# microsoft/foldingdiff

Measured on AMD Instinct MI355X. Metric: backbones/sec (L=128, T=1000, bs=512), higher is better.
Workload: dtype f32 (fp16 hi/lo split operands, 3x v_mfma_f32_{32x32x16,16x16x32}_f16 per product, fp32 accumulate)

## Files before the change

foldingdiff_amd/build.py:

```python
import os
import shutil
import subprocess
import sys
from concurrent.futures import ThreadPoolExecutor

PKG_DIR = os.path.dirname(os.path.abspath(__file__))
CSRC = os.path.join(PKG_DIR, "csrc")
LIB_DIR = os.path.join(PKG_DIR, "_lib")
LIB_PATH = os.path.join(LIB_DIR, "libfdmi.so")
SOURCES = ["api.hip", "api_weights.hip", "api_comm.hip", "api_run.hip", "api_structures.hip", "api_hooks.hip", "gemm_f32.hip", "gemm_img.hip", "gemm_ws.hip", "gemm_ln_rows.hip", "attention_f32.hip", "attention_img.hip", "attention_gen.hip", "seq_attn.hip", "seq_attn16.hip", "ffn16.hip", "rowwise.hip",
           "rowwise_img.hip", "inpaint_jump.hip", "loss.hip", "loss_variants.hip", "nerf.hip", "internal_coords.hip", "tm_score.hip", "psea.hip", "dssp.hip", "tm_align.hip", "tm_align_starts.hip", "clash_lddt.hip", "angle_stats.hip", "steer.hip", "repeat_tie.hip", "nerf_vjp.hip", "nerf_scan.hip", "relax.hip", "guide_scaffold.hip", "template_fit.hip"]
HEADERS = [os.path.join(CSRC, "fdmi_kernels.h"), os.path.join(CSRC, "img_common.h"), os.path.join(CSRC, "horn_fit.h"),
           os.path.join(CSRC, "launch_common.h"), os.path.join(CSRC, "host_common.h"), os.path.join(CSRC, "model.h"), os.path.join(CSRC, "weight_pack.h"), os.path.join(CSRC, "tm_search.h"), os.path.join(CSRC, "tm_align_common.h"), os.path.join(CSRC, "wrap_pi.h"), os.path.join(CSRC, "nerf_place.h"), os.path.join(CSRC, "smooth_l1_term.h"), os.path.join(CSRC, "philox_normal.h"), os.path.join(CSRC, "inpaint_replace.h"), os.path.join(CSRC, "strided_update.h"), os.path.join(CSRC, "solver_update.h"), os.path.join(CSRC, "p_sample_update.h"), os.path.join(CSRC, "block_sum.h"), os.path.join(CSRC, "guide_element.h"), os.path.join(os.path.dirname(PKG_DIR), "include", "fdmi.h")]
ARCH = "gfx950"
PER_SOURCE_FLAGS = {
    "attention_img": ["-fno-slp-vectorize"],
    "attention_gen": ["-fno-slp-vectorize"],
    "seq_attn": ["-fno-slp-vectorize"],
    "seq_attn16": ["-fno-slp-vectorize"],
    "ffn16": ["-fno-slp-vectorize"],
}
CXXFLAGS = ["-O3", "-std=c++17", "-fPIC", f"--offload-arch={ARCH}", "-Wall", "-Wno-unused-function"]


def find_hipcc() -> str:
    for cand in (os.environ.get("HIPCC"), shutil.which("hipcc"), "/opt/rocm/bin/hipcc"):
        if cand and os.path.exists(cand):
            return cand
    raise RuntimeError("hipcc not found (set HIPCC=/path/to/hipcc)")


def _stale(target: str, deps) -> bool:
    if not os.path.exists(target):
        return True
    t = os.path.getmtime(target)
    return any(os.path.getmtime(d) > t for d in deps)


def build(force: bool = False, verbose: bool = False, variant: str = "", defines=()) -> str:
    hipcc = find_hipcc()
    os.makedirs(LIB_DIR, exist_ok=True)
    lib_dir = os.path.join(LIB_DIR, variant) if variant else LIB_DIR
    lib_path = os.path.join(lib_dir, "libfdmi.so")
    obj_dir = os.path.join(lib_dir, "obj")
    os.makedirs(obj_dir, exist_ok=True)
    jobs = []
    objs = []
    revs = dict(d[4:].split("=", 1) for d in defines if d.startswith("rev:"))
    defines = [d for d in defines if not d.startswith("rev:")]
    old_sources = []
    for src in SOURCES:
        sp = os.path.join(CSRC, src)
        if src in revs:
# ... 6 lines not shown
        op = os.path.join(obj_dir, src.replace(".hip", ".o"))
        objs.append(op)
        if force or _stale(op, [sp] + HEADERS):
            stem = src.replace(".hip", "")
            extra = [d.split("=", 1)[1] for d in defines if d.startswith("@") and d[1:].split("=", 1)[0] in (stem, "all")]
            jobs.append([hipcc] + CXXFLAGS + PER_SOURCE_FLAGS.get(stem, []) + extra
                        + [f"-D{d}" for d in defines if not d.startswith("@")] + ["-c", sp, "-o", op])

    def run(cmd):
        if verbose:
            print(" ".join(cmd), flush=True)
        r = subprocess.run(cmd, capture_output=True, text=True)
        if r.returncode != 0:
            raise RuntimeError(f"hipcc failed ({r.returncode}):\n{' '.join(cmd)}\n{r.stdout}\n{r.stderr}")
        return r

    try:
        with ThreadPoolExecutor(max_workers=8) as ex:
            list(ex.map(run, jobs))
        counts = mfma_counts(defines, {src: os.path.join(CSRC, f"_rev_{variant}_{src}") for src in revs}) if variant else None
    finally:
        for sp in old_sources:
            os.remove(sp)
    if force or jobs or _stale(lib_path, objs):
        run([hipcc, f"--offload-arch={ARCH}", "-shared", "-fPIC"] + objs + ["-o", lib_path])
    if variant:
        import json
        meta = {"defines": list(defines), "revs": revs, "mfma": counts, "mfma_default": mfma_counts(())}
        with open(os.path.join(lib_dir, "build_info.json"), "w") as fh:
            json.dump(meta, fh, indent=1, sort_keys=True)
    return lib_path


MFMA_SOURCES = ["seq_attn16.hip", "ffn16.hip", "seq_attn.hip", "gemm_img.hip", "attention_img.hip"]


def mfma_counts(defines=(), paths=None) -> dict:
    import re
    import tempfile
    hipcc = find_hipcc()
    out = {}
    with tempfile.TemporaryDirectory() as td:
        for src in MFMA_SOURCES:
            stem = src.replace(".hip", "")
            extra = [d.split("=", 1)[1] for d in defines if d.startswith("@") and d[1:].split("=", 1)[0] in (stem, "all")]
            asm = os.path.join(td, stem + ".s")
            cmd = [hipcc, "-O3", "-std=c++17", f"--offload-arch={ARCH}", "-Wno-unused-function"] + PER_SOURCE_FLAGS.get(stem, []) + extra \
                + [f"-D{d}" for d in defines if not d.startswith("@")] + ["-S", "--cuda-device-only", "-o", asm, (paths or {}).get(src, os.path.join(CSRC, src))]
            r = subprocess.run(cmd, capture_output=True, text=True)
            if r.returncode != 0:
                raise RuntimeError(f"hipcc -S failed for {src}:\n{r.stderr[-2000:]}")
            text = open(asm).read()
            for m in re.finditer(r"^(_Z\w+):[^\n]*\n(.*?)^\.Lfunc_end\d+:", text, re.S | re.M):
                n = m.group(2).count("v_mfma")
                if n:
                    out[m.group(1)] = n
    return out


if __name__ == "__main__":
    args = [a for a in sys.argv[1:] if a != "--force"]
    p = build(force="--force" in sys.argv, verbose=True, variant=args[0] if args else "", defines=args[1:])
    print(p)
```

foldingdiff_amd/csrc/api.hip:

```cpp
#include <hip/hip_runtime.h>

#include <cstdarg>
#include <cstdio>
#include <cstring>
#include <string>
#include <utility>
#include <vector>

#include "../../include/fdmi.h"
#include "fdmi_kernels.h"
#include "host_common.h"
#include "launch_common.h"
#include "model.h"

using namespace fdmi;

namespace {
thread_local std::string g_err;
}

int fdmi::fail(int code, const char* fmt, ...) {
  char buf[1024];
  va_list ap;
  va_start(ap, fmt);
// ... 174 lines not shown
  m->pending.clear();
  return FD_OK;
}

#define PROF(cls, stmt)                                   \
  do {                                                    \
    int rc_ = prof_begin(m, cls, s, mode.profile);        \
    if (rc_) return rc_;                                  \
    stmt;                                                 \
    rc_ = prof_end(m, s, mode.profile);                   \
    if (rc_) return rc_;                                  \
  } while (0)

void prof_drop(fd_model* m, bool on) {
  if (!on) return;
  const PendingEvent p = m->pending.back();
  m->pending.pop_back();
  m->event_pool.push_back(p.e0);
  m->event_pool.push_back(p.e1);
}

struct EnvOverrides {
  int fuse_attn, fuse_ffn;
  bool stamps;
};
const EnvOverrides& env_overrides() {
  static const EnvOverrides env = [] {
    auto num = [](const char* name, int dflt) { const char* e = getenv(name); return e ? atoi(e) : dflt; };
    return EnvOverrides{num("FDMI_FUSE_ATTN", -1), num("FDMI_FUSE_FFN", -1), num("FDMI_STAMPS", 0) != 0};
  }();
  return env;
}

}

StepPlan fdmi::plan_step(const fd_model* m, const Workspace& w, bool key_mask, bool dyn_rows) {
  StepPlan p;
  p.img = w.img;
  if (!p.img) {
    p.fuse_ln = m->fuse_ln > 0;
    return p;
  }
  const fd_config& c = m->cfg;
  const LayerDev& lw = m->layers[0];
  const EnvOverrides& env = env_overrides();
  const int B = w.B, L = w.L, d = c.d_model, max_rows = w.cap, ncu = cu_count();
  auto whole_rounds = [&](int items) {
    const int rounds = (items + ncu - 1) / ncu;
    return (double)items >= 0.94 * (double)rounds * ncu;
  };
  const bool fits_u32 = (size_t)w.cap * d * 4 < (1ull << 32) - 65536;
  const int fuse_attn = m->fuse_attn >= 0 ? m->fuse_attn : env.fuse_attn;
  const bool attn_auto = !m->varlen && L > 96 && whole_rounds(B);
  const bool fused_ok = fuse_attn != 0 && (fuse_attn > 0 || attn_auto) && !key_mask && !m->split_qkv && fits_u32;
  if (fused_ok && fuse_attn != 2 && lw.wsa16_i.p && seq_attn16_supported(d, c.n_heads, L, c.max_pos)) p.attn = StepPlan::ATTN_FUSED16;
  else if (fused_ok && fuse_attn == 2 && lw.wsa_i.p && seq_attn_supported(d, c.n_heads, L, c.max_pos)) p.attn = StepPlan::ATTN_FUSED32;
  else p.attn = lw.wqkv_i.p && !m->split_qkv ? StepPlan::ATTN_QKV : StepPlan::ATTN_QK_VT;
  p.attn_gen = key_mask || head_dim(c) != 32;
  const int fuse_ffn = m->fuse_ffn >= 0 ? m->fuse_ffn : env.fuse_ffn;
  const int rows_known = m->varlen && m->rows_hint > 0 && m->rows_hint <= max_rows ? m->rows_hint : max_rows;
  const bool fused_ffn = fuse_ffn != 0 && (fuse_ffn > 0 || whole_rounds((rows_known + 127) / 128)) && lw.wff_i.p &&
                         ffn16_supported(d, c.d_ff) && fits_u32;
  p.ffn = !fused_ffn ? StepPlan::FFN_GEMMS : (fuse_ffn != 1 && lw.wtail_i.p && d <= 384) ? StepPlan::FFN_TAIL : StepPlan::FFN_FUSED;
  p.split_ln = d > 384;
  auto tail_for = [&](int N) {
    if (m->varlen || dyn_rows) return 1;
    const int ntiles = (max_rows / 128) * ((N + 383) / 384);
    return ntiles % gemm_img_grid(max_rows, N) != 0 ? 1 : 0;
  };
  if (!p.fused_attn()) p.tail_qk = tail_for(p.attn == StepPlan::ATTN_QKV ? 3 * d : 2 * d);
  p.tail_d = tail_for(d);
  if (p.ffn == StepPlan::FFN_GEMMS) p.tail_ff = tail_for(c.d_ff);
  return p;
}

namespace {

UpdateArgs fill_update(const fd_model* m, const Workspace& w, const StepMode& mode) {
  UpdateArgs u;
  memset(&u, 0, sizeof u);
  if (m->cfg.decoder == FD_DEC_MLP) {
    u.gamma = m->hd_g;
    u.beta = m->hd_b;
    u.do_ln = 1;
  }
  u.w2 = m->hd_w2;
  u.b2 = m->hd_b2;
  u.x = w.x;
  u.coef = m->coef;
  u.t_dev = w.t_dev;
  u.T = m->T;
  u.M = w.B * w.L;
  u.L = w.L;
  u.F = m->cfg.n_features;
  u.d = m->cfg.d_model;
  u.ln_eps = 1e-12f;
// ... 157 lines not shown
        PROF(KC_GEMM_QKV, launch_gemm_img(EPI_IMG_QK, g, max_rows, s));
        if (stop_after(1)) return done();
        g = base();
        g.A = w.himg; g.W = static_cast<const unsigned char*>(lw.wv_i.p); g.bias = lw.bv;
        g.vbuf = w.vbuf; g.N = d; g.K = d;
        g.acc_scale = 1.0f / (lw.s_h * lw.wv_i.scale); g.v_scale = lw.s_v;
        g.tail = plan.tail_d;
        PROF(KC_GEMM_V, launch_gemm_img(EPI_IMG_VT, g, max_rows, s));
        if (stop_after(1)) return done();
      }
      AttnImgArgs a;
      memset(&a, 0, sizeof a);
      a.qbuf = w.qbuf; a.kbuf = w.kbuf; a.vbuf = w.vbuf;
      a.demb = static_cast<const u32x4_t*>(lw.demb_s.p);
      a.lens = w.lens; a.nrow = w.nrow; a.seq_row0 = w.seq_row0; a.ctx = w.cimg; a.trash = w.trash;
      a.B = B; a.H = H; a.LTOT = w.LTOT; a.NKT = w.NKT; a.maxpos = c.max_pos;
      a.q_scale = lw.s_q; a.k_scale = lw.s_k; a.v_scale = lw.s_v; a.ctx_scale = lw.s_v;
      a.r_scale = lw.demb_s.p ? lw.s_k / lw.demb_s.scale : 1.f;
      a.r_scale_k = lw.demb_s.p ? lw.s_q / lw.demb_s.scale : 1.f;
      a.rkq = c.pos_type == FD_POS_RELATIVE_KEY_QUERY;
      a.stamps = stamps_at(kStampAttn);
      bool ok = true;
      if (plan.attn_gen) {
        a.H = c.n_heads;
        a.kmask = mode.kmask;
        a.L = mode.kmask ? L : 0;
        PROF(KC_ATTN, ok = launch_attention_gen(a, head_dim(c) / 32, s));
      } else {
        PROF(KC_ATTN, ok = launch_attention_img(a, L, s));
      }
      if (!ok) return fail(FD_E_UNSUPPORTED, "attention: L=%d, head size %d", L, head_dim(c));
      if (stop_after(1)) return done();
    }
    const bool fused_tail = plan.ffn == StepPlan::FFN_TAIL;
    if (!fused_tail) {
      GemmImgArgs g = base();
      g.A = w.cimg; g.W = static_cast<const unsigned char*>(lw.wo_i.p); g.bias = lw.bo; g.gamma = lw.ln1g; g.beta = lw.ln1b;
      g.resid = w.himg; g.out = w.aimg; g.K = d;
      g.acc_scale = 1.0f / (lw.s_v * lw.wo_i.scale); g.resid_inv = 1.0f / lw.s_h; g.out_scale = lw.s_a;
      if (int rc = gemm_ln(g, KC_GEMM_OUT, KC_LN1)) return rc;
      if (stop_after(1)) return done();
    }
    if (plan.ffn != StepPlan::FFN_GEMMS) {
      FfnArgs a;
      memset(&a, 0, sizeof a);
      a.aimg = w.aimg; a.a_bytes = (unsigned)((size_t)w.cap * d * 4);
      a.wimg = static_cast<const unsigned char*>(fused_tail ? lw.wtail_i.p : lw.wff_i.p);
      if (fused_tail) {
        a.cimg = w.cimg; a.hres = w.himg; a.bo = lw.bo; a.g1 = lw.ln1g; a.b1 = lw.ln1b;
        a.ao_scale = 1.0f / (lw.s_v * lw.wtail_i.scale); a.hres_inv = 1.0f / lw.s_h; a.a_scale = lw.s_a; a.eps1 = c.ln_eps;
      }
      a.bi = lw.bi; a.bd = lw.bd; a.gamma = lw.ln2g; a.beta = lw.ln2b;
      a.out = w.himg; a.out_bytes = a.a_bytes;
      a.panels = max_rows / 128; a.dims = w.dims;
      a.up_scale = 1.0f / (lw.s_a * lw.wff_i.scale); a.g_scale = lw.s_g; a.down_scale = 1.0f / (lw.s_g * lw.wff_scale_dn);
      a.resid_inv = 1.0f / lw.s_a; a.out_scale = s_next; a.eps = c.ln_eps;
      a.stamps = stamps_at(kStampFfn);
      bool launched = false;
      PROF(fused_tail ? KC_TAIL : KC_FFN, launched = launch_ffn16(a, d, s, m->debug_grid, &w.grids[2]));
      if (!launched) return fail(FD_E_HIP, "the fused feed-forward kernel could not be launched");
      if (stop_after(fused_tail ? 3 : 2)) return done();
      continue;
    }
    {
      GemmImgArgs g = base();
      g.A = w.aimg; g.W = static_cast<const unsigned char*>(lw.wi_i.p); g.bias = lw.bi; g.out = w.gimg; g.N = ff; g.K = d;
      g.acc_scale = 1.0f / (lw.s_a * lw.wi_i.scale); g.out_scale = lw.s_g;
      g.tail = plan.tail_ff;
      PROF(KC_GEMM_UP, launch_gemm_img(EPI_IMG_GELU, g, max_rows, s));
      if (stop_after(1)) return done();
    }
    {
      GemmImgArgs g = base();
      g.A = w.gimg; g.W = static_cast<const unsigned char*>(lw.wd_i.p); g.bias = lw.bd; g.gamma = lw.ln2g; g.beta = lw.ln2b;
      g.resid = w.aimg; g.out = w.himg; g.K = ff;
      g.acc_scale = 1.0f / (lw.s_g * lw.wd_i.scale); g.resid_inv = 1.0f / lw.s_a; g.out_scale = s_next;
      if (int rc = gemm_ln(g, KC_GEMM_DOWN, KC_LN2)) return rc;
      if (stop_after(1)) return done();
    }
  }
  UpdateArgs u = fill_update(m, w, mode);
  HeadImgArgs hi;
  memset(&hi, 0, sizeof hi);
  if (c.decoder == FD_DEC_MLP) {
    GemmImgArgs g = base();
    g.A = w.himg; g.W = static_cast<const unsigned char*>(m->hd_w1_i.p); g.bias = m->hd_b1; g.out = w.gimg; g.N = d; g.K = d;
    g.acc_scale = 1.0f / (m->s_hfinal * m->hd_w1_i.scale); g.out_scale = m->s_hg;
    g.tail = plan.tail_d;
    PROF(KC_GEMM_HEAD, launch_gemm_img(EPI_IMG_GELU, g, max_rows, s));
    if (stop_after(1)) return done();
    hi.g = w.gimg; hi.g_inv = 1.0f / m->s_hg;
  } else {
// ... 133 lines not shown
  m->device = device_id;
  hipError_t e = hipStreamCreateWithFlags(&m->stream, hipStreamNonBlocking);
  if (e != hipSuccess) {
    delete m;
    return fail(FD_E_HIP, "hipStreamCreate: %s", hipGetErrorString(e));
  }
  *out = m;
  return FD_OK;
}

void fd_destroy(fd_model* m) {
  if (!m) return;
  (void)hipSetDevice(m->device);
  (void)fd_comm_destroy(m);
  if (m->stream) (void)hipStreamSynchronize(m->stream);
  drop_workspaces(m);
  free_weights(m);
  for (PendingEvent& p : m->pending) {
    (void)hipEventDestroy(p.e0);
    (void)hipEventDestroy(p.e1);
  }
  for (hipEvent_t e : m->event_pool) (void)hipEventDestroy(e);
  if (m->stream) (void)hipStreamDestroy(m->stream);
  delete m;
}

int fd_set_option(fd_model* m, const char* name, int value) {
  if (!m || !name) return fail(FD_E_INVALID, "null argument");
  const std::string n = name;
  if (n == "fuse_ln") m->fuse_ln = value < 0 ? -1 : (value ? 1 : 0);
  else if (n == "use_graph") m->use_graph = value ? 1 : 0;
  else if (n == "varlen") m->varlen = value ? 1 : 0;
  else if (n == "fuse_attn") m->fuse_attn = value < 0 ? -1 : (value > 2 ? 1 : value);
  else if (n == "fuse_ffn") m->fuse_ffn = value < 0 ? -1 : (value > 2 ? 2 : value);
  else if (n == "rows_hint") m->rows_hint = value < 0 ? 0 : value;
  else if (n == "split_qkv") {
    m->split_qkv = value ? 1 : 0;
    drop_workspaces(m);
  }
  else if (n == "debug_stop") {
    if (m->debug_stop != value) drop_workspaces(m);
    m->debug_stop = value;
  }
  else if (n == "debug_layer") m->debug_layer = value;
  else if (n == "debug_grid") {
    const int v = value > 0 ? value : 0;
    if (m->debug_grid != v) drop_workspaces(m);
    m->debug_grid = v;
  }
  else return fail(FD_E_INVALID, "unknown option '%s'", name);
  return FD_OK;
}

int fd_fused_attn_supported(fd_model* m, int L) {
  if (!m) return fail(FD_E_INVALID, "null argument");
  if (!m->finalized) return fail(FD_E_STATE, "fd_finalize has not been called");
  if (m->precision != FD_PREC_F16X3 || m->layers.empty() || L < 1) return 0;
  const fd_config& c = m->cfg;
  const LayerDev& lw = m->layers[0];
  if (m->fuse_attn == 2) return lw.wsa_i.p && seq_attn_supported(c.d_model, c.n_heads, L, c.max_pos) ? 1 : 0;
  return lw.wsa16_i.p && seq_attn16_supported(c.d_model, c.n_heads, L, c.max_pos) ? 1 : 0;
}

int fd_profile_every(fd_model* m, int n) {
  if (!m || n < 0) return fail(FD_E_INVALID, "bad argument");
  m->profile_every = n;
  return FD_OK;
// ... 119 lines not shown
```

foldingdiff_amd/csrc/fdmi_kernels.h:

```cpp
#pragma once
#include <hip/hip_runtime.h>
#include <stdint.h>

namespace fdmi {

constexpr int kHeadDim = 32;
constexpr int kMaxFeat = 16;
typedef unsigned u32x4_t __attribute__((ext_vector_type(4)));

enum GemmEpilogue {
  EPI_BIAS = 0,
  EPI_BIAS_GELU = 1,
  EPI_BIAS_RESID = 2
};

void launch_gemm_f32(int epilogue, const float* A, const float* W, const float* bias, const float* resid, float* C,
                     int M, int N, int K, hipStream_t s);

bool launch_gemm_f32_ln(const float* A, const float* W, const float* bias, const float* resid, const float* gamma,
                        const float* beta, float eps, float* C, int M, int N, int K, hipStream_t s);

void launch_layernorm(const float* x, const float* gamma, const float* beta, float eps, float* y, int rows, int d,
                      hipStream_t s);

// ... 294 lines not shown
bool launch_seq_attn16(const SeqAttnArgs& p, hipStream_t s, int grid_cap = 0, int* grid_used = nullptr);

struct FfnArgs {
  const unsigned char* aimg;
  unsigned a_bytes;
  const unsigned char* wimg;
  const float* bi;
  const float* bd;
  const float* gamma;
  const float* beta;
  unsigned char* out;
  unsigned out_bytes;
  int panels;
  const int* dims;
  float up_scale;
  float g_scale;
  float down_scale;
  float resid_inv;
  float out_scale;
  float eps;
  const unsigned char* cimg;
  const unsigned char* hres;
  const float* bo;
  const float* g1;
  const float* b1;
  float ao_scale;
  float hres_inv;
  float a_scale;
  float eps1;
  unsigned long long* stamps;
};
bool ffn16_supported(int d_model, int d_ff);
bool launch_ffn16(const FfnArgs& p, int d_model, hipStream_t s, int grid_cap = 0, int* grid_used = nullptr);

struct EmbedImgArgs {
  const float* x;
  const float* w_in; const float* b_in; const float* pos_emb; const float* gamma; const float* beta;
  const float* time_table;
  int* tslot;
  const int2* rowinfo; const int* nrow; const int* dims;
  const int* pos_ids;
  unsigned char* h;
  int L, F, d;
  float eps, out_scale;
};
void launch_embed_img(const EmbedImgArgs& a, const int* t_seq, int max_rows, hipStream_t s, bool ar = false);
void launch_ar_step(float* x, const float* eps, int B, int L, int F, int copy_pos, int rows_next, int cap, int* lens, int* nrow,
                    int* seq_row0, int2* rowinfo, int* dims, hipStream_t s);

struct HeadImgArgs {
  const unsigned char* g;
  float g_inv;
  const int2* rowinfo; const int* nrow; const int* dims;
  int* tslot;
  int* flag;
  int advance;
};
void launch_head_update_img(const UpdateArgs& a, const HeadImgArgs& ia, int max_rows, hipStream_t s);

void launch_ln_f32_img(const float* src, const float* gamma, const float* beta, float eps, const int* dims, void* out, int d,
                       float out_scale, int max_rows, hipStream_t s);

struct ShiftTrimArgs {
  const float* traj;
  const int* lens;
  const long long* item_off;
// ... 56 lines not shown
```

foldingdiff_amd/csrc/model.h:

```cpp
#pragma once
#include <hip/hip_runtime.h>

#include <cstdint>
#include <map>
#include <string>
#include <tuple>
#include <vector>

#include "../../include/fdmi.h"
#include "fdmi_kernels.h"

namespace fdmi {

struct HostTensor {
  std::vector<float> data;
  std::vector<int64_t> shape;
};

struct SplitW {
  void* p = nullptr;
  float scale = 1.f;
};

struct LayerDev {
  SplitW demb_s;
  SplitW wqk_i, wv_i, wqkv_i, wo_i, wi_i, wd_i;
  SplitW wsa_i;
  SplitW wff_i;
  float wff_scale_dn = 1.f;
  SplitW wtail_i;
  SplitW wsa16_i;
  float *bqk = nullptr, *bv = nullptr;
  float s_h = 1.f, s_q = 1.f, s_k = 1.f, s_v = 1.f, s_a = 1.f, s_g = 1.f;
  float *wqkv = nullptr, *bqkv = nullptr, *demb = nullptr;
  float *wo = nullptr, *bo = nullptr, *ln1g = nullptr, *ln1b = nullptr;
  float *wi = nullptr, *bi = nullptr, *wd = nullptr, *bd = nullptr, *ln2g = nullptr, *ln2b = nullptr;
};

enum KClass {
  KC_EMBED = 0, KC_GEMM_QKV, KC_GEMM_V, KC_ATTN, KC_GEMM_OUT, KC_LN1, KC_GEMM_UP, KC_GEMM_DOWN, KC_LN2, KC_GEMM_HEAD,
  KC_HEAD_UPDATE, KC_ADVANCE, KC_SEQ_ATTN, KC_FFN, KC_TAIL, KC_COUNT
};
const char* const kClassName[KC_COUNT] = {
    "embed_ln_time", "gemm_qkv", "gemm_v", "attention", "gemm_attn_out", "layernorm_attn", "gemm_ffn_up",
    "gemm_ffn_down", "layernorm_ffn", "gemm_head_dense1", "head_update_wrap", "step_advance", "qkv_attention_fused", "ffn_fused", "attn_out_ffn_fused"};

struct StepPlan {
  enum Attn { ATTN_QKV, ATTN_QK_VT, ATTN_FUSED16, ATTN_FUSED32 };
  enum Ffn { FFN_GEMMS, FFN_FUSED, FFN_TAIL };
  bool img = false;
  bool fuse_ln = false;
  int attn = ATTN_QKV;
  bool attn_gen = false;
  int ffn = FFN_GEMMS;
  bool split_ln = false;
  int tail_qk = 0, tail_d = 0, tail_ff = 0;
  bool fused_attn() const { return attn == ATTN_FUSED16 || attn == ATTN_FUSED32; }
  bool operator==(const StepPlan& o) const {
    return std::tie(img, fuse_ln, attn, attn_gen, ffn, split_ln, tail_qk, tail_d, tail_ff) ==
           std::tie(o.img, o.fuse_ln, o.attn, o.attn_gen, o.ffn, o.split_ln, o.tail_qk, o.tail_d, o.tail_ff);
  }
};

struct Workspace {
  int B = 0, L = 0;
  float *x = nullptr, *eps = nullptr, *h = nullptr, *qkv = nullptr, *ctx = nullptr, *a = nullptr, *tmp = nullptr,
        *g = nullptr, *z = nullptr;
  int* lens = nullptr;
  int* t_dev = nullptr;
  int* t_seq = nullptr;
  float* loss_in = nullptr;
  double* loss_sums = nullptr;
  float* loss_ex_in = nullptr;
  double* loss_ex_out = nullptr;
  UpdateDyn* dyn = nullptr;
  float* inpaint = nullptr;
  bool img = false;
  int cap = 0, LPK = 0, LTOT = 0, NKT = 0;
  unsigned char *himg = nullptr, *aimg = nullptr, *cimg = nullptr, *gimg = nullptr, *qbuf = nullptr, *kbuf = nullptr,
                *vbuf = nullptr, *trash = nullptr;
  int2* rowinfo = nullptr;
  int *seq_row0 = nullptr, *nrow = nullptr, *dims = nullptr, *flag = nullptr;
  unsigned char* kmask = nullptr;
  int* pos_ids = nullptr;
  int grids[3] = {0, 0, 0};
  hipGraphExec_t graph = nullptr;
  StepPlan graph_plan;
  uint64_t last_use = 0;
  void release() {
    if (graph) (void)hipGraphExecDestroy(graph);
    graph = nullptr;
    for (void* p : {(void*)x, (void*)eps, (void*)h, (void*)qkv, (void*)ctx, (void*)a, (void*)tmp, (void*)g, (void*)z,
                    (void*)lens, (void*)t_dev, (void*)t_seq, (void*)loss_in, (void*)loss_sums, (void*)loss_ex_in, (void*)loss_ex_out, (void*)dyn, (void*)inpaint, (void*)himg, (void*)aimg, (void*)cimg, (void*)gimg,
// ... 105 lines not shown
```

Measured before the change: 82.76.

## Add streaming fused FFN tail kernel with triple-buffered weight staging

Adds a new persistent FFN-tail kernel specialised for d_model=384, d_ff=768. It streams the weight image through a three-stage LDS ring using buffer-to-LDS DMA, overlapped with 16x16x32 fp16 MFMA work and next-panel context prefetch. The planner selects it automatically when supported, falling back to the existing fused FFN kernel if the launch fails. The aim is to hide weight-load latency inside the feed-forward tail, at the cost of a large hand-scheduled kernel with heavy register and LDS pressure.

```diff
diff --git a/foldingdiff_amd/build.py b/foldingdiff_amd/build.py
--- a/foldingdiff_amd/build.py
+++ b/foldingdiff_amd/build.py
@@ -8,7 +8,7 @@
 CSRC = os.path.join(PKG_DIR, "csrc")
 LIB_DIR = os.path.join(PKG_DIR, "_lib")
 LIB_PATH = os.path.join(LIB_DIR, "libfdmi.so")
-SOURCES = ["api.hip", "api_weights.hip", "api_comm.hip", "api_run.hip", "api_structures.hip", "api_hooks.hip", "gemm_f32.hip", "gemm_img.hip", "gemm_ws.hip", "gemm_ln_rows.hip", "attention_f32.hip", "attention_img.hip", "attention_gen.hip", "seq_attn.hip", "seq_attn16.hip", "ffn16.hip", "rowwise.hip",
+SOURCES = ["api.hip", "api_weights.hip", "api_comm.hip", "api_run.hip", "api_structures.hip", "api_hooks.hip", "gemm_f32.hip", "gemm_img.hip", "gemm_ws.hip", "gemm_ln_rows.hip", "attention_f32.hip", "attention_img.hip", "attention_gen.hip", "seq_attn.hip", "seq_attn16.hip", "ffn16.hip", "ffn16_stream.hip", "rowwise.hip",
            "rowwise_img.hip", "inpaint_jump.hip", "loss.hip", "loss_variants.hip", "nerf.hip", "internal_coords.hip", "tm_score.hip", "psea.hip", "dssp.hip", "tm_align.hip", "tm_align_starts.hip", "clash_lddt.hip", "angle_stats.hip", "steer.hip", "repeat_tie.hip", "nerf_vjp.hip", "nerf_scan.hip", "relax.hip", "guide_scaffold.hip", "template_fit.hip"]
 HEADERS = [os.path.join(CSRC, "fdmi_kernels.h"), os.path.join(CSRC, "img_common.h"), os.path.join(CSRC, "horn_fit.h"),
            os.path.join(CSRC, "launch_common.h"), os.path.join(CSRC, "host_common.h"), os.path.join(CSRC, "model.h"), os.path.join(CSRC, "weight_pack.h"), os.path.join(CSRC, "tm_search.h"), os.path.join(CSRC, "tm_align_common.h"), os.path.join(CSRC, "wrap_pi.h"), os.path.join(CSRC, "nerf_place.h"), os.path.join(CSRC, "smooth_l1_term.h"), os.path.join(CSRC, "philox_normal.h"), os.path.join(CSRC, "inpaint_replace.h"), os.path.join(CSRC, "strided_update.h"), os.path.join(CSRC, "solver_update.h"), os.path.join(CSRC, "p_sample_update.h"), os.path.join(CSRC, "block_sum.h"), os.path.join(CSRC, "guide_element.h"), os.path.join(os.path.dirname(PKG_DIR), "include", "fdmi.h")]
@@ -19,6 +19,7 @@
     "seq_attn": ["-fno-slp-vectorize"],
     "seq_attn16": ["-fno-slp-vectorize"],
     "ffn16": ["-fno-slp-vectorize"],
+    "ffn16_stream": ["-fno-slp-vectorize"],
 }
 CXXFLAGS = ["-O3", "-std=c++17", "-fPIC", f"--offload-arch={ARCH}", "-Wall", "-Wno-unused-function"]
 
@@ -91,7 +92,7 @@
     return lib_path
 
 
-MFMA_SOURCES = ["seq_attn16.hip", "ffn16.hip", "seq_attn.hip", "gemm_img.hip", "attention_img.hip"]
+MFMA_SOURCES = ["seq_attn16.hip", "ffn16.hip", "ffn16_stream.hip", "seq_attn.hip", "gemm_img.hip", "attention_img.hip"]
 
 
 def mfma_counts(defines=(), paths=None) -> dict:
diff --git a/foldingdiff_amd/csrc/api.hip b/foldingdiff_amd/csrc/api.hip
--- a/foldingdiff_amd/csrc/api.hip
+++ b/foldingdiff_amd/csrc/api.hip
@@ -230,6 +230,8 @@
   return env;
 }
 
+constexpr bool kStreamTailAuto = true;
+
 }
 
 StepPlan fdmi::plan_step(const fd_model* m, const Workspace& w, bool key_mask, bool dyn_rows) {
@@ -260,6 +262,13 @@
   const bool fused_ffn = fuse_ffn != 0 && (fuse_ffn > 0 || whole_rounds((rows_known + 127) / 128)) && lw.wff_i.p &&
                          ffn16_supported(d, c.d_ff) && fits_u32;
   p.ffn = !fused_ffn ? StepPlan::FFN_GEMMS : (fuse_ffn != 1 && lw.wtail_i.p && d <= 384) ? StepPlan::FFN_TAIL : StepPlan::FFN_FUSED;
+  if (p.ffn == StepPlan::FFN_TAIL && ffn16_stream_supported(d, c.d_ff)) {
+    if (fuse_ffn == 3) p.ffn = StepPlan::FFN_TAIL_STREAM;
+    else if (fuse_ffn < 0 && kStreamTailAuto && ffn16_stream_ready()) {
+      p.ffn = StepPlan::FFN_TAIL_STREAM;
+      p.ffn_auto = true;
+    }
+  }
   p.split_ln = d > 384;
   auto tail_for = [&](int N) {
     if (m->varlen || dyn_rows) return 1;
@@ -483,7 +492,8 @@
       if (!ok) return fail(FD_E_UNSUPPORTED, "attention: L=%d, head size %d", L, head_dim(c));
       if (stop_after(1)) return done();
     }
-    const bool fused_tail = plan.ffn == StepPlan::FFN_TAIL;
+    const bool stream_tail = plan.ffn == StepPlan::FFN_TAIL_STREAM;
+    const bool fused_tail = plan.ffn == StepPlan::FFN_TAIL || stream_tail;
     if (!fused_tail) {
       GemmImgArgs g = base();
       g.A = w.cimg; g.W = static_cast<const unsigned char*>(lw.wo_i.p); g.bias = lw.bo; g.gamma = lw.ln1g; g.beta = lw.ln1b;
@@ -508,7 +518,12 @@
       a.resid_inv = 1.0f / lw.s_a; a.out_scale = s_next; a.eps = c.ln_eps;
       a.stamps = stamps_at(kStampFfn);
       bool launched = false;
-      PROF(fused_tail ? KC_TAIL : KC_FFN, launched = launch_ffn16(a, d, s, m->debug_grid, &w.grids[2]));
+      if (stream_tail) {
+        PROF(KC_TAIL, launched = launch_ffn16_stream(a, s, m->debug_grid, &w.grids[2]));
+        if (!launched && plan.ffn_auto) prof_drop(m, mode.profile);
+      }
+      if (!launched && (!stream_tail || plan.ffn_auto))
+        PROF(fused_tail ? KC_TAIL : KC_FFN, launched = launch_ffn16(a, d, s, m->debug_grid, &w.grids[2]));
       if (!launched) return fail(FD_E_HIP, "the fused feed-forward kernel could not be launched");
       if (stop_after(fused_tail ? 3 : 2)) return done();
       continue;
@@ -708,7 +723,7 @@
   else if (n == "use_graph") m->use_graph = value ? 1 : 0;
   else if (n == "varlen") m->varlen = value ? 1 : 0;
   else if (n == "fuse_attn") m->fuse_attn = value < 0 ? -1 : (value > 2 ? 1 : value);
-  else if (n == "fuse_ffn") m->fuse_ffn = value < 0 ? -1 : (value > 2 ? 2 : value);
+  else if (n == "fuse_ffn") m->fuse_ffn = value < 0 ? -1 : (value > 3 ? 3 : value);
   else if (n == "rows_hint") m->rows_hint = value < 0 ? 0 : value;
   else if (n == "split_qkv") {
     m->split_qkv = value ? 1 : 0;
diff --git a/foldingdiff_amd/csrc/fdmi_kernels.h b/foldingdiff_amd/csrc/fdmi_kernels.h
--- a/foldingdiff_amd/csrc/fdmi_kernels.h
+++ b/foldingdiff_amd/csrc/fdmi_kernels.h
@@ -350,6 +350,9 @@
 };
 bool ffn16_supported(int d_model, int d_ff);
 bool launch_ffn16(const FfnArgs& p, int d_model, hipStream_t s, int grid_cap = 0, int* grid_used = nullptr);
+bool ffn16_stream_supported(int d_model, int d_ff);
+bool ffn16_stream_ready();
+bool launch_ffn16_stream(const FfnArgs& p, hipStream_t s, int grid_cap = 0, int* grid_used = nullptr);
 
 struct EmbedImgArgs {
   const float* x;
diff --git a/foldingdiff_amd/csrc/ffn16_stream.hip b/foldingdiff_amd/csrc/ffn16_stream.hip
--- /dev/null
+++ b/foldingdiff_amd/csrc/ffn16_stream.hip
@@ -0,0 +1,516 @@
+#include <cstdlib>
+#include <type_traits>
+
+#include "fdmi_kernels.h"
+#include "img_common.h"
+#include "launch_common.h"
+
+namespace fdmi {
+namespace ffns {
+
+typedef float f32x4 __attribute__((ext_vector_type(4)));
+typedef const __attribute__((address_space(3))) u32x4* lds_cu128_t;
+typedef __attribute__((address_space(3))) u32x4* lds_u128_t;
+__device__ __forceinline__ unsigned lds_addr(const void* p) { return (unsigned)(unsigned long long)(lds_ptr_t)(const_cast<void*>(p)); }
+__device__ __forceinline__ u32x4 lds_u128(unsigned a) { return *(lds_cu128_t)(unsigned long long)a; }
+__device__ __forceinline__ f16x8 lds_f16x8(unsigned a) { return __builtin_bit_cast(f16x8, lds_u128(a)); }
+__device__ __forceinline__ void lds_put128(unsigned a, const u32x4& v) { *(lds_u128_t)(unsigned long long)a = v; }
+
+__device__ __forceinline__ void swap16(unsigned& vdst, unsigned& src) {
+  const auto r = __builtin_amdgcn_permlane16_swap(vdst, src, false, false);
+  vdst = r[0];
+  src = r[1];
+}
+__device__ __forceinline__ float quad_sum(float x) {
+  unsigned a = __builtin_bit_cast(unsigned, x), b = a;
+  swap32(a, b);
+  float m = __builtin_bit_cast(float, a) + __builtin_bit_cast(float, b);
+  a = __builtin_bit_cast(unsigned, m);
+  b = a;
+  swap16(a, b);
+  return __builtin_bit_cast(float, a) + __builtin_bit_cast(float, b);
+}
+
+template <int V> using IC = std::integral_constant<int, V>;
+template <int LO, int HI, class F>
+__device__ __forceinline__ void static_for(F&& f) {
+  if constexpr (LO < HI) {
+    f(IC<LO>{});
+    static_for<LO + 1, HI>(f);
+  }
+}
+
+#ifndef FDMI_FFN_PRIO
+#define FDMI_FFN_PRIO 2
+#endif
+
+__device__ __forceinline__ f32x4 mfma16(const f16x8& a, const f16x8& b, const f32x4& c) {
+  return __builtin_amdgcn_mfma_f32_16x16x32_f16(a, b, c, 0, 0, 0);
+}
+
+constexpr int NKT = 12;
+constexpr int D = 32 * NKT;
+constexpr int NW = 8;
+constexpr int TILE = 2048;
+constexpr int STEP = 4 * TILE;
+constexpr int SPS = 2;
+constexpr int STAGE = SPS * STEP;
+constexpr int NST = 3;
+constexpr int PPW = STAGE / 1024 / NW;
+constexpr int OFF_W = 0;
+constexpr int OFF_X = NST * STAGE;
+constexpr int OFF_P = OFF_X + NW * NKT * 1024;
+constexpr int OFF_P1 = OFF_P + 5 * D * 4;
+constexpr int SMEM = OFF_P + 8 * D * 4;
+constexpr int NG = NKT;
+constexpr int SPG = 2 * NKT;
+constexpr int STG = SPG / SPS;
+constexpr int NSA = NKT * NKT / 2;
+constexpr int BPS = NKT / 2;
+constexpr int W_BYTES = (NSA / SPS + NG * STG) * STAGE;
+constexpr int CTX_FIRST = 2;
+
+__host__ __device__ constexpr int rows_requested(int b) { return b <= NKT - 2 ? 4 : 0; }
+__host__ __device__ constexpr int top_wait(int s) { return s % BPS == 1 ? PPW : PPW + rows_requested(s / BPS); }
+__host__ __device__ constexpr int res_step(int r) {
+  constexpr int o[BPS] = {3, 4, 5, 2, 3, 2};
+  return r == NKT - 1 ? BPS * (NKT - 1) + 3 : BPS * (r + 1) + o[r / 2];
+}
+
+template <bool PROF>
+__global__ __launch_bounds__(64 * NW) void ffn16_kernel_stream(FfnArgs p) {
+  extern __shared__ __attribute__((aligned(16))) unsigned char smem[];
+  const int tid = threadIdx.x, lane = tid & 63;
+  const int wq = __builtin_amdgcn_readfirstlane(tid >> 6);
+  const int grp = wq >> 2;
+  unsigned smem0 = __builtin_amdgcn_readfirstlane(lds_addr(smem));
+  asm volatile("" : "+s"(smem0));
+  auto lane_id = [&]() __attribute__((always_inline)) {
+    int ln;
+    asm volatile("v_mbcnt_lo_u32_b32 %0, -1, 0\n\tv_mbcnt_hi_u32_b32 %0, -1, %0" : "=v"(ln));
+    return ln;
+  };
+  auto lane_off_of = [](int ln) __attribute__((always_inline)) { return (unsigned)((ln >> 4) * 256 + (ln & 15) * 16); };
+
+  {
+    float* par = reinterpret_cast<float*>(smem + OFF_P);
+    for (int i = tid; i < 2 * D; i += 64 * NW) par[i] = p.bi[i];
+    for (int i = tid; i < D; i += 64 * NW) {
+      par[2 * D + i] = p.bd[i];
+      par[3 * D + i] = p.gamma[i];
+      par[4 * D + i] = p.beta[i] * p.out_scale;
+      par[5 * D + i] = p.bo[i] * (1.0f / p.ao_scale);
+      par[6 * D + i] = p.g1[i];
+      par[7 * D + i] = p.b1[i] * p.a_scale;
+    }
+  }
+
+  int w_src = 0, w_slot = 0;
+  const __amdgpu_buffer_rsrc_t rs_w = __builtin_amdgcn_make_buffer_rsrc(const_cast<unsigned char*>(p.wimg), 0, W_BYTES, 0x00020000);
+  auto issue_w = [&]() __attribute__((always_inline)) {
+    const lds_ptr_t dst = (lds_ptr_t)(unsigned long long)(smem0 + OFF_W + (unsigned)__builtin_amdgcn_readfirstlane(w_slot));
+    const int so = __builtin_amdgcn_readfirstlane(w_src);
+    const int vo = lane_id() * 16;
+#pragma unroll
+    for (int k = 0; k < PPW; ++k) dma16(rs_w, dst + (wq + NW * k) * 1024, vo, so + (wq + NW * k) * 1024);
+    w_src = w_src + STAGE == W_BYTES ? 0 : w_src + STAGE;
+    w_slot = w_slot + STAGE == NST * STAGE ? 0 : w_slot + STAGE;
+  };
+
+  f16x8 ah[NKT];
+  u32x4 tl[NKT];
+  u32x4 rh[NKT], rl[NKT];
+  const __amdgpu_buffer_rsrc_t rs_a = __builtin_amdgcn_make_buffer_rsrc(const_cast<unsigned char*>(p.cimg), 0, p.a_bytes, 0x00020000);
+  const __amdgpu_buffer_rsrc_t rs_h = __builtin_amdgcn_make_buffer_rsrc(const_cast<unsigned char*>(p.hres), 0, p.a_bytes, 0x00020000);
+  auto row_off = [&](int r0) __attribute__((always_inline)) {
+    const int ln = lane_id();
+    const int row = r0 + 16 * wq + (ln & 15);
+    return (unsigned)(((row >> 5) * (NKT * 256) + (row & 31)) * 16 + (ln >> 4) * 512);
+  };
+  auto load_ctx = [&](auto KT, unsigned hoff) __attribute__((always_inline)) {
+    constexpr int kt = decltype(KT)::value;
+    ah[kt] = __builtin_bit_cast(f16x8, __builtin_amdgcn_raw_buffer_load_b128(rs_a, (int)hoff, kt * 8 * 512, 0));
+    tl[kt] = __builtin_bit_cast(u32x4, __builtin_amdgcn_raw_buffer_load_b128(rs_a, (int)hoff, (kt * 8 + 4) * 512, 0));
+  };
+  auto commit_lo = [&](auto KT) __attribute__((always_inline)) {
+    constexpr int kt = decltype(KT)::value;
+    lds_put128(smem0 + OFF_X + (unsigned)(wq * NKT * 1024 + lane_id() * 16 + kt * 1024), tl[kt]);
+  };
+  auto load_res = [&](auto KT, unsigned hoff) __attribute__((always_inline)) {
+    constexpr int kt = decltype(KT)::value;
+    rh[kt] = __builtin_bit_cast(u32x4, __builtin_amdgcn_raw_buffer_load_b128(rs_h, (int)hoff, kt * 8 * 512, 0));
+    rl[kt] = __builtin_bit_cast(u32x4, __builtin_amdgcn_raw_buffer_load_b128(rs_h, (int)hoff, (kt * 8 + 4) * 512, 0));
+  };
+  const __amdgpu_buffer_rsrc_t rs_o = __builtin_amdgcn_make_buffer_rsrc(p.out, 0, p.out_bytes, 0x00020000);
+
+  const bool rec = PROF && blockIdx.x == 0 && p.stamps != nullptr;
+  unsigned long long* stp = PROF ? p.stamps + (size_t)wq * 16 * 16 : nullptr;
+  int slot = 0;
+#define FD_STAMP(i) do { if (PROF) { if (rec && slot < 15 && lane == 0) stp[slot * 16 + (i)] = __builtin_amdgcn_s_memtime(); } } while (0)
+#define FD_SB() __builtin_amdgcn_sched_barrier(0)
+#define FD_STAMP_G(i) do { if (PROF) { if (rec && slot == 0 && G == 1 && lane == 0) stp[15 * 16 + (i)] = __builtin_amdgcn_s_memtime(); } } while (0)
+
+  const int n_pass = p.dims ? min(p.panels, __builtin_amdgcn_readfirstlane(p.dims[1]) >> 7) : p.panels;
+  if ((int)blockIdx.x >= n_pass) return;
+  const float os_up = p.up_scale, os_dn = p.down_scale, hs = 0.5f * p.g_scale;
+  const f32x4 zero4 = {0.f, 0.f, 0.f, 0.f};
+  f32x4 Y[2 * NKT];
+  f32x4 U[4];
+  f32x4 Up[4];
+  u32x4 uh[2], ul[2];
+
+  {
+    const unsigned hoff = row_off((int)blockIdx.x * 128);
+    static_for<0, CTX_FIRST>([&](auto KT) __attribute__((always_inline)) { load_ctx(KT, hoff); });
+  }
+  issue_w();
+  issue_w();
+  issue_w();
+  FD_WAIT_VM(3 * PPW);
+  static_for<0, CTX_FIRST>([&](auto KT) __attribute__((always_inline)) { commit_lo(KT); });
+  FD_WAIT_VM(2 * PPW);
+  barrier_keep_vm();
+
+  auto gelu_piece = [&](auto P, unsigned abq) __attribute__((always_inline)) {
+    constexpr int pc = decltype(P)::value, pr = pc >> 2, j = pc & 3;
+    const u32x2 b = *(const __attribute__((address_space(3))) u32x2*)(unsigned long long)(abq + (unsigned)((32 * pr + 2 * j) * 4));
+    float o0 = __builtin_fmaf(Up[2 * pr + (j >> 1)][2 * (j & 1)], os_up, __builtin_bit_cast(float, (unsigned)b[0]));
+    float o1 = __builtin_fmaf(Up[2 * pr + (j >> 1)][2 * (j & 1) + 1], os_up, __builtin_bit_cast(float, (unsigned)b[1]));
+    const float h0 = o0 * hs, h1 = o1 * hs;
+    o0 = __builtin_fmaf(h0, erf_rational(o0 * 0.70710678118654752440f), h0);
+    o1 = __builtin_fmaf(h1, erf_rational(o1 * 0.70710678118654752440f), h1);
+    unsigned a, c;
+    split_pair(o0, o1, a, c);
+    uh[pr][j] = a;
+    ul[pr][j] = c;
+  };
+
+  auto add_res = [&](auto R) __attribute__((always_inline)) {
+    constexpr int r = decltype(R)::value;
+    const unsigned pb1 = smem0 + OFF_P1 + (unsigned)(8 * (lane_id() >> 4) * 4);
+    const float c = p.hres_inv * (1.0f / p.ao_scale);
+    const u32x4 b0 = lds_u128(pb1 + (unsigned)(r * 128)), b1 = lds_u128(pb1 + (unsigned)(r * 128 + 16));
+#pragma unroll
+    for (int j = 0; j < 2; ++j)
+#pragma unroll
+      for (int e = 0; e < 4; e += 2) {
+        const unsigned hw = rh[r][2 * j + e / 2], lw = rl[r][2 * j + e / 2];
+        const unsigned bw0 = j == 0 ? b0[e] : b1[e], bw1 = j == 0 ? b0[e + 1] : b1[e + 1];
+        const float v0 = fma_mix_lo(hw, c, __builtin_bit_cast(float, bw0));
+        const float v1 = fma_mix_hi(hw, c, __builtin_bit_cast(float, bw1));
+        Y[2 * r + j][e] += fma_mix_lo(lw, c, v0);
+        Y[2 * r + j][e + 1] += fma_mix_hi(lw, c, v1);
+      }
+  };
+
+  auto steps = [&](auto S0, auto S1, auto GEL, unsigned abq, unsigned hoff) __attribute__((always_inline)) {
+    constexpr int s0 = decltype(S0)::value, s1 = decltype(S1)::value;
+    constexpr bool gel = decltype(GEL)::value == 1, pha = decltype(GEL)::value == 2;
+    auto stage_top = [&]() __attribute__((always_inline)) {
+      FD_WAIT_VM(PPW);
+      barrier_keep_vm();
+      issue_w();
+    };
+    f16x8 fx[4], fy[4], xl;
+    unsigned a_W, a_X;
+    {
+      const int ln = lane_id();
+      a_W = smem0 + OFF_W + lane_off_of(ln);
+      a_X = smem0 + OFF_X + (unsigned)(wq * NKT * 1024 + ln * 16);
+      asm volatile("" : "+v"(a_W), "+v"(a_X));
+    }
+    auto plane_reads = [&](auto S, auto LO, f16x8 (&f)[4]) __attribute__((always_inline)) {
+      constexpr int s = decltype(S)::value, lo = decltype(LO)::value;
+      constexpr unsigned off = (unsigned)(((s / SPS) % NST) * STAGE + (s % SPS) * STEP + lo * 1024);
+#pragma unroll
+      for (int t = 0; t < 4; ++t) f[t] = lds_f16x8(a_W + off + (unsigned)(t * TILE));
+      if constexpr (pha) {
+        if constexpr (lo == 0 && s % BPS == 0) xl = lds_f16x8(a_X + (unsigned)((s / BPS) * 1024));
+      } else {
+        if constexpr (lo == 0 && s < NKT) xl = lds_f16x8(a_X + (unsigned)(s * 1024));
+      }
+    };
+    auto mm = [&](auto S, auto WHICH, const f16x8 (&f)[4]) __attribute__((always_inline)) {
+      constexpr int s = decltype(S)::value, which = decltype(WHICH)::value;
+      if constexpr (pha) {
+        constexpr int kt = s / BPS, q = s % BPS;
+#pragma unroll
+        for (int t = 0; t < 4; ++t) Y[4 * q + t] = mfma16(f[t], which == 1 ? xl : ah[kt], Y[4 * q + t]);
+      } else if constexpr (s < NKT) {
+#pragma unroll
+        for (int t = 0; t < 4; ++t) U[t] = mfma16(f[t], which == 1 ? xl : ah[s], U[t]);
+      } else {
+        constexpr int pr = (s - NKT) / (NKT / 2), q = (s - NKT) % (NKT / 2);
+#pragma unroll
+        for (int t = 0; t < 4; ++t) Y[4 * q + t] = mfma16(f[t], __builtin_bit_cast(f16x8, which == 1 ? ul[pr] : uh[pr]), Y[4 * q + t]);
+      }
+    };
+    plane_reads(S0, IC<0>{}, fx);
+    FD_SB();
+    static_for<s0, s1>([&](auto S) __attribute__((always_inline)) {
+      constexpr int s = decltype(S)::value;
+      constexpr bool top = s % SPS == SPS - 1;
+      plane_reads(S, IC<1>{}, fy);
+      FD_SB();
+      if constexpr (top) {
+        if constexpr (pha) {
+          FD_WAIT_VM(top_wait(s));
+          if (grp == 0) barrier_keep_vm();
+        } else {
+          if (grp == 0) stage_top();
+        }
+      }
+#if FDMI_FFN_PRIO
+      __builtin_amdgcn_s_setprio(FDMI_FFN_PRIO);
+#endif
+      mm(S, IC<0>{}, fx);
+      mm(S, IC<1>{}, fx);
+#if FDMI_FFN_PRIO
+      __builtin_amdgcn_s_setprio(0);
+#endif
+      FD_SB();
+      if constexpr (pha && s == 0) {
+        FD_STAMP(15);
+        FD_SB();
+      }
+      if constexpr (top) {
+        if constexpr (pha) {
+          if (grp != 0) barrier_keep_vm();
+          issue_w();
+        } else {
+          if (grp != 0) stage_top();
+        }
+      }
+      if constexpr (pha && s % BPS == 1) {
+        constexpr int b = s / BPS;
+        if constexpr (b >= 1 && b + 1 < NKT) {
+          commit_lo(IC<b + 1>{});
+        }
+        if constexpr (b + CTX_FIRST < NKT) {
+          load_ctx(IC<b + CTX_FIRST>{}, hoff);
+          load_res(IC<b>{}, hoff);
+        } else if constexpr (b == NKT - 2) {
+          load_res(IC<NKT - 2>{}, hoff);
+          load_res(IC<NKT - 1>{}, hoff);
+        }
+        FD_SB();
+      }
+      if constexpr (s + 1 < s1) plane_reads(IC<s + 1>{}, IC<0>{}, fx);
+      FD_SB();
+      if constexpr (gel) {
+        if (grp == 0) {
+          static_for<0, 8>([&](auto P) __attribute__((always_inline)) {
+            if constexpr (1 + decltype(P)::value * (NKT - 2) / 8 == s) gelu_piece(P, abq);
+          });
+        }
+        FD_SB();
+      }
+      mm(S, IC<2>{}, fy);
+      FD_SB();
+      if constexpr (gel) {
+        if (grp != 0) {
+          static_for<0, 8>([&](auto P) __attribute__((always_inline)) {
+            if constexpr (1 + decltype(P)::value * (NKT - 2) / 8 == s) gelu_piece(P, abq);
+          });
+        }
+        FD_SB();
+      }
+      if constexpr (pha) {
+        static_for<0, NKT>([&](auto R) __attribute__((always_inline)) {
+          if constexpr (res_step(decltype(R)::value) == s) {
+            add_res(R);
+            FD_SB();
+          }
+        });
+      }
+    });
+  };
+
+  for (int panel = blockIdx.x; panel < n_pass; panel += (int)gridDim.x) {
+    FD_STAMP(0);
+    {
+#pragma unroll
+      for (int t = 0; t < 2 * NKT; ++t) Y[t] = zero4;
+      steps(IC<0>{}, IC<NSA>{}, IC<2>{}, 0u, row_off(panel * 128));
+      const int ln = lane_id();
+      const int g = ln >> 4;
+      const unsigned pb1 = smem0 + OFF_P1 + (unsigned)(8 * g * 4);
+      const unsigned ax = smem0 + OFF_X + (unsigned)(wq * NKT * 1024 + ln * 16);
+      const float os_ao = p.ao_scale;
+      float sum = 0.f;
+#pragma unroll
+      for (int t = 0; t < 2 * NKT; ++t)
+#pragma unroll
+        for (int e = 0; e < 4; ++e) {
+          Y[t][e] *= os_ao;
+          sum += Y[t][e];
+        }
+      const float inv_n = 1.0f / (float)D;
+      float mean = quad_sum(sum) * inv_n;
+      asm volatile("" : "+v"(mean));
+      float t2 = 0.f;
+#pragma unroll
+      for (int t = 0; t < 2 * NKT; ++t)
+#pragma unroll
+        for (int e = 0; e < 4; ++e) {
+          const float dl = Y[t][e] - mean;
+          Y[t][e] = dl;
+          t2 = __builtin_fmaf(dl, dl, t2);
+        }
+      const float rstd = (1.0f / sqrtf(__builtin_fmaf(quad_sum(t2), inv_n, p.eps1))) * p.a_scale;
+#pragma unroll
+      for (int kt = 0; kt < NKT; ++kt) {
+        const u32x4 g0 = lds_u128(pb1 + (unsigned)(D * 4 + kt * 128)), g1 = lds_u128(pb1 + (unsigned)(D * 4 + kt * 128 + 16));
+        const u32x4 e0 = lds_u128(pb1 + (unsigned)(2 * D * 4 + kt * 128)), e1 = lds_u128(pb1 + (unsigned)(2 * D * 4 + kt * 128 + 16));
+        float o[8];
+#pragma unroll
+        for (int e = 0; e < 4; ++e) {
+          o[e] = __builtin_fmaf(Y[2 * kt][e] * rstd, __builtin_bit_cast(float, (unsigned)g0[e]), __builtin_bit_cast(float, (unsigned)e0[e]));
+          o[4 + e] = __builtin_fmaf(Y[2 * kt + 1][e] * rstd, __builtin_bit_cast(float, (unsigned)g1[e]), __builtin_bit_cast(float, (unsigned)e1[e]));
+        }
+        u32x4 hv, lv;
+#pragma unroll
+        for (int j = 0; j < 4; ++j) {
+          unsigned a, b;
+          split_pair(o[2 * j], o[2 * j + 1], a, b);
+          hv[j] = a;
+          lv[j] = b;
+        }
+        ah[kt] = __builtin_bit_cast(f16x8, hv);
+        lds_put128(ax + (unsigned)(kt * 1024), lv);
+      }
+    }
+#pragma unroll
+    for (int t = 0; t < 2 * NKT; ++t) Y[t] = zero4;
+#pragma unroll
+    for (int t = 0; t < 4; ++t) U[t] = zero4;
+    steps(IC<0>{}, IC<NKT>{}, IC<0>{}, 0u, 0u);
+    for (int G = 0; G < NG; ++G) {
+#pragma unroll
+      for (int t = 0; t < 4; ++t) {
+        Up[t] = U[t];
+        U[t] = zero4;
+      }
+      unsigned abq = smem0 + OFF_P + (unsigned)((64 * G + 8 * (lane_id() >> 4)) * 4);
+      asm volatile("" : "+v"(abq));
+      FD_STAMP_G(0);
+      FD_STAMP_G(1);
+      if (G + 1 < NG) {
+        steps(IC<0>{}, IC<NKT>{}, IC<1>{}, abq, 0u);
+      } else {
+        static_for<0, 8>([&](auto P) __attribute__((always_inline)) { gelu_piece(P, abq); });
+      }
+      FD_STAMP_G(2);
+      steps(IC<NKT>{}, IC<SPG>{}, IC<0>{}, 0u, 0u);
+      FD_STAMP_G(3);
+      if (slot == 0) FD_STAMP(1 + (G < 12 ? G : 11));
+    }
+    {
+      const int ln = lane_id();
+      const int g = ln >> 4;
+      const unsigned pb = smem0 + OFF_P + (unsigned)((2 * D + 8 * g) * 4);
+      const unsigned ax = smem0 + OFF_X + (unsigned)(wq * NKT * 1024 + ln * 16);
+      const float ri = p.resid_inv;
+      float sum = 0.f;
+#pragma unroll
+      for (int kt = 0; kt < NKT; ++kt) {
+        const u32x4 b0 = lds_u128(pb + (unsigned)(kt * 128)), b1 = lds_u128(pb + (unsigned)(kt * 128 + 16));
+        const u32x4 rhv = __builtin_bit_cast(u32x4, ah[kt]), rlv = lds_u128(ax + (unsigned)(kt * 1024));
+#pragma unroll
+        for (int j = 0; j < 2; ++j)
+#pragma unroll
+          for (int e = 0; e < 4; e += 2) {
+            const unsigned bw0 = j == 0 ? b0[e] : b1[e], bw1 = j == 0 ? b0[e + 1] : b1[e + 1];
+            float v0 = __builtin_fmaf(Y[2 * kt + j][e], os_dn, __builtin_bit_cast(float, bw0));
+            float v1 = __builtin_fmaf(Y[2 * kt + j][e + 1], os_dn, __builtin_bit_cast(float, bw1));
+            const unsigned hw = rhv[2 * j + e / 2], lw = rlv[2 * j + e / 2];
+            v0 = fma_mix_lo(hw, ri, v0);
+            v1 = fma_mix_hi(hw, ri, v1);
+            v0 = fma_mix_lo(lw, ri, v0);
+            v1 = fma_mix_hi(lw, ri, v1);
+            Y[2 * kt + j][e] = v0;
+            Y[2 * kt + j][e + 1] = v1;
+            sum += v0;
+            sum += v1;
+          }
+      }
+      const int next = panel + (int)gridDim.x;
+      {
+        const unsigned noff = row_off(next * 128);
+        static_for<0, CTX_FIRST>([&](auto KT) __attribute__((always_inline)) { load_ctx(KT, noff); });
+      }
+      const float inv_n = 1.0f / (float)D;
+      float mean = quad_sum(sum) * inv_n;
+      asm volatile("" : "+v"(mean));
+      float t2 = 0.f;
+#pragma unroll
+      for (int t = 0; t < 2 * NKT; ++t)
+#pragma unroll
+        for (int e = 0; e < 4; ++e) {
+          const float dl = Y[t][e] - mean;
+          Y[t][e] = dl;
+          t2 = __builtin_fmaf(dl, dl, t2);
+        }
+      const float rstd = (1.0f / sqrtf(__builtin_fmaf(quad_sum(t2), inv_n, p.eps))) * p.out_scale;
+      const unsigned ooff = row_off(panel * 128);
+      static_for<0, NKT>([&](auto KT) __attribute__((always_inline)) {
+        constexpr int kt = decltype(KT)::value;
+        const u32x4 g0 = lds_u128(pb + (unsigned)(D * 4 + kt * 128)), g1 = lds_u128(pb + (unsigned)(D * 4 + kt * 128 + 16));
+        const u32x4 e0 = lds_u128(pb + (unsigned)(2 * D * 4 + kt * 128)), e1 = lds_u128(pb + (unsigned)(2 * D * 4 + kt * 128 + 16));
+        float o[8];
+#pragma unroll
+        for (int e = 0; e < 4; ++e) {
+          o[e] = __builtin_fmaf(Y[2 * kt][e] * rstd, __builtin_bit_cast(float, (unsigned)g0[e]), __builtin_bit_cast(float, (unsigned)e0[e]));
+          o[4 + e] = __builtin_fmaf(Y[2 * kt + 1][e] * rstd, __builtin_bit_cast(float, (unsigned)g1[e]), __builtin_bit_cast(float, (unsigned)e1[e]));
+        }
+        u32x4 hv, lv;
+#pragma unroll
+        for (int j = 0; j < 4; ++j) {
+          unsigned a, b;
+          split_pair(o[2 * j], o[2 * j + 1], a, b);
+          hv[j] = a;
+          lv[j] = b;
+        }
+        __builtin_amdgcn_raw_buffer_store_b128(hv, rs_o, (int)ooff, kt * 8 * 512, 0);
+        __builtin_amdgcn_raw_buffer_store_b128(lv, rs_o, (int)ooff, (kt * 8 + 4) * 512, 0);
+        store_guard(hv, lv);
+        FD_SB();
+      });
+    }
+    FD_STAMP(13);
+    FD_WAIT_VM(0);
+    static_for<0, CTX_FIRST>([&](auto KT) __attribute__((always_inline)) { commit_lo(KT); });
+    FD_STAMP(14);
+    ++slot;
+  }
+  FD_WAIT_VM(0);
+#undef FD_STAMP
+#undef FD_STAMP_G
+#undef FD_SB
+}
+
+static LdsOptIn& lds_opt_in() {
+  static LdsOptIn lds;
+  return lds;
+}
+static bool opt_in() {
+  return lds_opt_in()({reinterpret_cast<const void*>(&ffn16_kernel_stream<false>), reinterpret_cast<const void*>(&ffn16_kernel_stream<true>)}, SMEM);
+}
+
+}
+
+bool ffn16_stream_supported(int d_model, int d_ff) { return d_model == 384 && d_ff == 768; }
+
+bool ffn16_stream_ready() { return ffns::opt_in(); }
+
+bool launch_ffn16_stream(const FfnArgs& p, hipStream_t s, int grid_cap, int* grid_used) {
+  if (!p.cimg || !ffns::opt_in()) return false;
+  const int grid = persistent_grid(p.panels, grid_cap);
+  if (grid <= 0) return true;
+  if (grid_used) *grid_used = grid;
+  if (p.stamps) hipLaunchKernelGGL((ffns::ffn16_kernel_stream<true>), dim3(grid), dim3(64 * ffns::NW), ffns::SMEM, s, p);
+  else hipLaunchKernelGGL((ffns::ffn16_kernel_stream<false>), dim3(grid), dim3(64 * ffns::NW), ffns::SMEM, s, p);
+  return hipGetLastError() == hipSuccess;
+}
+
+}
diff --git a/foldingdiff_amd/csrc/model.h b/foldingdiff_amd/csrc/model.h
--- a/foldingdiff_amd/csrc/model.h
+++ b/foldingdiff_amd/csrc/model.h
@@ -47,18 +47,19 @@
 
 struct StepPlan {
   enum Attn { ATTN_QKV, ATTN_QK_VT, ATTN_FUSED16, ATTN_FUSED32 };
-  enum Ffn { FFN_GEMMS, FFN_FUSED, FFN_TAIL };
+  enum Ffn { FFN_GEMMS, FFN_FUSED, FFN_TAIL, FFN_TAIL_STREAM };
   bool img = false;
   bool fuse_ln = false;
   int attn = ATTN_QKV;
   bool attn_gen = false;
   int ffn = FFN_GEMMS;
+  bool ffn_auto = false;
   bool split_ln = false;
   int tail_qk = 0, tail_d = 0, tail_ff = 0;
   bool fused_attn() const { return attn == ATTN_FUSED16 || attn == ATTN_FUSED32; }
   bool operator==(const StepPlan& o) const {
-    return std::tie(img, fuse_ln, attn, attn_gen, ffn, split_ln, tail_qk, tail_d, tail_ff) ==
-           std::tie(o.img, o.fuse_ln, o.attn, o.attn_gen, o.ffn, o.split_ln, o.tail_qk, o.tail_d, o.tail_ff);
+    return std::tie(img, fuse_ln, attn, attn_gen, ffn, ffn_auto, split_ln, tail_qk, tail_d, tail_ff) ==
+           std::tie(o.img, o.fuse_ln, o.attn, o.attn_gen, o.ffn, o.ffn_auto, o.split_ln, o.tail_qk, o.tail_d, o.tail_ff);
   }
 };
 
```

New measurement: 82.51. About the same (-0.3%).
